# XuehuaOvO/MPC_via_Diffusion_Model

Hardware: AMD Instinct MI355X
Metric: candidate trajectories/sec (100 denoise steps, H=32) (higher is better)
Workload: dtype f32

## Files before the change

### include/mpcd.h

```cpp
#ifndef MPCD_H
#define MPCD_H

#include <stddef.h>
#include <stdint.h>

#ifdef __cplusplus
extern "C" {
#endif

typedef struct mpcd_ctx mpcd_ctx;

enum mpcd_status {
    MPCD_OK = 0,
    MPCD_EINVAL = -1,
    MPCD_EHIP = -2,
    MPCD_ESTATE = -3,
    MPCD_ENOMEM = -4,
    MPCD_EUNSUP = -5,
    MPCD_ENONFINITE = -6,
};

enum mpcd_net_kind {
    MPCD_NET_MLP = 1,
    MPCD_NET_UNET = 2,
// ... 5 lines not shown
    int32_t kind;
    int32_t state_dim;
    int32_t horizon;
    int32_t context_dim;
    int32_t base_dim;
    int32_t n_mults;
    int32_t mults[4];
    int32_t time_emb_dim;
    int32_t cfg_masked;
    int32_t dtype;
} mpcd_net_desc;

int mpcd_net_param_count(const mpcd_net_desc *desc, int32_t *n_tensors, int64_t *n_floats);
int mpcd_net_param_info(const mpcd_net_desc *desc, int32_t i, char *name, size_t name_cap,
                        int32_t *ndim, int64_t shape[4]);

int mpcd_create(int device, mpcd_ctx **out);
void mpcd_destroy(mpcd_ctx *ctx);
const char *mpcd_last_error(void);

int mpcd_load_net(mpcd_ctx *ctx, const mpcd_net_desc *desc, const float *blob_host, size_t n_floats);

int mpcd_set_schedule(mpcd_ctx *ctx, const float *tables_host, int32_t n_steps, const float *posterior_std_host);

enum mpcd_sampler {
    MPCD_DDPM_CFG = 0,
    MPCD_DDIM_CFG = 1,
    MPCD_DDIM = 2,
};

// ... 313 lines not shown
```

### mpc_via_diffusion_model_amd/_native.py

```python
import ctypes
import os

import torch

_HERE = os.path.dirname(os.path.abspath(__file__))
LIB_PATH = os.environ.get("MPCD_LIB") or os.path.join(_HERE, "libmpcd.so")

MPCD_NET_MLP, MPCD_NET_UNET = 1, 2
MPCD_F32, MPCD_F16, MPCD_F32X3, MPCD_F16X2 = 0, 1, 2, 3
MPCD_DDPM_CFG, MPCD_DDIM_CFG, MPCD_DDIM = 0, 1, 2
MPCD_COST_CANONICAL, MPCD_COST_CALMPC = 0, 1
MPCD_COMM_ID_BYTES = 128
MPCD_MAX_ELITES = 64
MPCD_CLIP_CHAIN, MPCD_CLIP_FINAL, MPCD_CLIP_NONE = 0, 1, 2

_STATUS = {-1: "EINVAL", -2: "EHIP", -3: "ESTATE", -4: "ENOMEM", -5: "EUNSUP", -6: "ENONFINITE"}
MPCD_ENONFINITE = -6
MPCD_STEP_CLIPPED, MPCD_STEP_NAN_SAMPLES, MPCD_STEP_NONFINITE_WINNER, MPCD_STEP_F32X3_RERUN = 1, 2, 4, 8
MPCD_STEP_INFEASIBLE = 16
MPCD_MAX_CON_ROWS = 8


class NetDesc(ctypes.Structure):
    _fields_ = [("kind", ctypes.c_int32), ("state_dim", ctypes.c_int32), ("horizon", ctypes.c_int32),
# ... 91 lines not shown
                ("reserved", ctypes.c_int32), ("next_priors_out", ctypes.c_void_p), ("elites_host", ctypes.c_void_p),
                ("elite_viol_host", ctypes.c_void_p), ("viol_host", ctypes.POINTER(ctypes.c_double)),
                ("n_feasible_host", ctypes.POINTER(ctypes.c_int64))]


class TrainCfg(ctypes.Structure):
    _fields_ = [("lr", ctypes.c_float), ("beta1", ctypes.c_float), ("beta2", ctypes.c_float), ("eps", ctypes.c_float),
                ("ema_decay", ctypes.c_float), ("step_start_ema", ctypes.c_int32), ("update_ema_every", ctypes.c_int32)]


EXPORTS = {
    "mpcd_net_param_count": ([ctypes.POINTER(NetDesc), ctypes.POINTER(ctypes.c_int32), ctypes.POINTER(ctypes.c_int64)],
                             ctypes.c_int),
    "mpcd_net_param_info": ([ctypes.POINTER(NetDesc), ctypes.c_int32, ctypes.c_char_p, ctypes.c_size_t,
                             ctypes.POINTER(ctypes.c_int32), ctypes.POINTER(ctypes.c_int64)], ctypes.c_int),
    "mpcd_create": ([ctypes.c_int, ctypes.POINTER(ctypes.c_void_p)], ctypes.c_int),
    "mpcd_destroy": ([ctypes.c_void_p], None),
    "mpcd_last_error": ([], ctypes.c_char_p),
    "mpcd_load_net": ([ctypes.c_void_p, ctypes.POINTER(NetDesc), ctypes.c_void_p, ctypes.c_size_t], ctypes.c_int),
    "mpcd_set_schedule": ([ctypes.c_void_p, ctypes.c_void_p, ctypes.c_int32, ctypes.c_void_p], ctypes.c_int),
    "mpcd_sample_steps": ([ctypes.c_void_p, ctypes.POINTER(SampleArgs), ctypes.POINTER(ctypes.c_int32)], ctypes.c_int),
    "mpcd_sample": ([ctypes.c_void_p, ctypes.POINTER(SampleArgs), ctypes.c_void_p], ctypes.c_int),
    "mpcd_sample_grouped": ([ctypes.c_void_p, ctypes.POINTER(SampleArgs), ctypes.c_int64, ctypes.c_void_p], ctypes.c_int),
    "mpcd_sample_warm": ([ctypes.c_void_p, ctypes.POINTER(SampleArgs), ctypes.c_int64, ctypes.POINTER(WarmStart),
                          ctypes.c_void_p], ctypes.c_int),
    "mpcd_sample_steps_warm": ([ctypes.c_void_p, ctypes.POINTER(SampleArgs), ctypes.POINTER(WarmStart),
                                ctypes.POINTER(ctypes.c_int32)], ctypes.c_int),
    "mpcd_shift_plans": ([ctypes.c_void_p, ctypes.c_void_p, ctypes.c_int64, ctypes.c_int32, ctypes.c_void_p,
                          ctypes.c_int64, ctypes.c_int64, ctypes.c_void_p, ctypes.c_void_p], ctypes.c_int),
    "mpcd_mpc_step_warm": ([ctypes.c_void_p, ctypes.POINTER(StepArgs), ctypes.POINTER(WarmStart), ctypes.c_void_p,
# ... 141 lines not shown
```

### mpc_via_diffusion_model_amd/csrc/internal.h

```cpp
#pragma once
#include <hip/hip_ext.h>
#include <hip/hip_runtime.h>
#include <stdint.h>

#include <mutex>

#include "../../include/mpcd.h"
#include "common.h"

struct CondLayer {
    const float *W;
    const float *b;
    int32_t width;
    int32_t off;
};

void launch_time_prologue(const StepPlan *plan, int n_steps, const float *time_w1, const float *time_b1,
                          const float *time_w2, const float *time_b2, const CondLayer *layers_dev, int n_layers,
                          int cond_dim, int cond_total, float *tproj, hipStream_t stream);

void launch_ctx_prologue(const float *ctx, int64_t n_rows, int ctx_dim, const CondLayer *layers_dev, int n_layers,
                         int cond_dim, int cond_total, float *cproj, hipStream_t stream);
void launch_ctx_replicate(const float *src, int64_t batch, int64_t group, int cond_total, float *dst, hipStream_t stream);
constexpr int kCtxRowMax = 64;
// ... 61 lines not shown
    uint64_t seed;
    int32_t n_steps;
    int32_t mode;
    int32_t clamp_x0;
    float wp1, wf;
    float *dbg;
    int32_t ctx_fused;
    int32_t ctx_dim, n_cond, cond_dim;
    const CondLayer *cond_layers;
    CtxRowArg ctx_row;
    int64_t group;
    int32_t group_wgs;
    int32_t x_init_kind;
    const float *x_init;
    float x_sa, x_sb;
};

int mlp_packed_floats(int d0);
void mlp_pack_weights(int d0, const float *const *lin_w, const float *const *lin_b, float *out);
hipError_t launch_mlp_sampler(int d0, int nb, const MlpSampleArgs &a, hipStream_t stream);
int mlp_packed_floats_x3(int d0);
void mlp_x3_force_layout(int layout);
int mlp_x3_layout_of(int64_t batch, int nb);
int mlp_x3_layout_grouped(int64_t n_groups, int64_t group, int nb);
void mlp_pack_weights_x3(int d0, const float *const *lin_w, const float *const *lin_b, float *out);
hipError_t launch_mlp_x3(int d0, int nb, const MlpSampleArgs &a, hipStream_t stream);
hipError_t launch_mlp_rw(int d0, int rows, int waves, const MlpSampleArgs &a, hipStream_t stream);
bool mlp_h2_supports(int d0, int mode);
int mlp_packed_floats_h2(int d0);
void mlp_pack_weights_h2(int d0, const float *const *lin_w, const float *const *lin_b, float *out);
hipError_t launch_mlp_h2(int d0, int rows, const MlpSampleArgs &a, hipStream_t stream);
// ... 117 lines not shown
```

### mpc_via_diffusion_model_amd/csrc/mlp_common.h

```cpp
#pragma once
#include <hip/hip_runtime.h>
#include <stdint.h>

#include <type_traits>

#include "common.h"

namespace mlpc {

constexpr int NLAYER = 14;
constexpr int COND_TOTAL = 448;
enum { EPI_NONE = 0, EPI_MISH = 1, EPI_CMISH = 2 };
constexpr int MODE_DDPM_XN = 16;

template <int D0>
struct Arch {
    static constexpr int K[NLAYER] = {D0, 32, 32, 64, 64, 128, 128, 128, 256, 64, 128, 32, 32, 32};
    static constexpr int N[NLAYER] = {32, 32, 64, 64, 128, 128, 128, 128, 64, 64, 32, 32, 32, D0};
    __host__ __device__ static constexpr int woff(int l) {
        int o = 0;
        for (int i = 0; i < l; ++i) o += K[i] * N[i] + N[i];
        return o;
    }
    static constexpr int total() { return woff(NLAYER); }
// ... 3 lines not shown
        return o;
    }
    static constexpr int total3() { return woff3(NLAYER); }
    __host__ __device__ static constexpr int boff(int l) {
        int o = 0;
        for (int i = 0; i < l; ++i) o += N[i];
        return o;
    }
    static constexpr int btotal() { return boff(NLAYER); }
};

inline int layer_k(int d0, int l) { return l == 0 ? d0 : Arch<32>::K[l]; }
inline int layer_n(int d0, int l) { return l == NLAYER - 1 ? d0 : Arch<32>::N[l]; }

__host__ __device__ constexpr int cond_off(int j) { return j == 0 ? 0 : j == 1 ? 32 : j == 2 ? 96 : j == 3 ? 224 : j == 4 ? 352 : 416; }

MPCD_DEV StepPlan load_plan(const StepPlan *plan, int s)
{
    typedef const __attribute__((address_space(4))) StepPlan *cplan_t;
    const cplan_t q = (cplan_t)(uintptr_t)plan + s;
    StepPlan r;
    r.t = q->t;
    r.flags = q->flags;
    r.a = q->a;
    r.b = q->b;
    r.c1 = q->c1;
    r.c2 = q->c2;
    r.std = q->std;
    r.sqan = q->sqan;
    r.cn = q->cn;
// ... 152 lines not shown
```

### mpc_via_diffusion_model_amd/csrc/mlp_rw.hip

```cpp
#include <hip/hip_runtime.h>

#include "mlp_x3.h"

namespace {
using namespace mlpx3;
static_assert(WPL == 3, "mlp_rw streams the three-plane pack");

constexpr int RW_W = 4;
constexpr int RW_T = 64 * RW_W;
constexpr int RES_L0 = 5;
constexpr int RES_NL = 3;
constexpr int RES_G = RES_NL * 2 * 4;
constexpr int RES_AG = 21;
constexpr int RES_AG8 = 10;

MPCD_DEV f32x2 exp2_pair(f32x2 z)
{
    float a, b;
    asm("v_exp_f32 %0, %2\n\tv_exp_f32 %1, %3\n\ts_nop 1" : "=&v"(a), "=&v"(b) : "v"(z[0]), "v"(z[1]));
    return f32x2{a, b};
}
MPCD_DEV f32x2 rcp_pair(f32x2 x)
{
    float a, b;
    asm("v_rcp_f32 %0, %2\n\tv_rcp_f32 %1, %3\n\ts_nop 1" : "=&v"(a), "=&v"(b) : "v"(x[0]), "v"(x[1]));
    return f32x2{a, b};
}
MPCD_DEV f32x2 fma2(f32x2 a, f32x2 b, f32x2 c) { return __builtin_elementwise_fma(a, b, c); }

constexpr int wpl(int m) { return m == 0 ? 2 : (m == 1 || m == 3) ? 1 : 0; }
constexpr int xpl(int m) { return (m == 0 || m == 3 || m == 5) ? 0 : (m == 1 || m == 4) ? 1 : 2; }

template <bool FIRST, bool LAST>
MPCD_DEV f32x4 mfma_agpr1(const u32x4 &w, const u32x4 &x, f32x4 acc)
{
    if constexpr (FIRST && LAST)
        asm("s_nop 1\n\tv_mfma_f32_16x16x32_bf16 %0, %1, %2, %0\n\ts_nop 7" : "+v"(acc) : "a"(w), "v"(x));
    else if constexpr (FIRST)
        asm("s_nop 1\n\tv_mfma_f32_16x16x32_bf16 %0, %1, %2, %0" : "+v"(acc) : "a"(w), "v"(x));
    else if constexpr (LAST)
        asm("v_mfma_f32_16x16x32_bf16 %0, %1, %2, %0\n\ts_nop 7" : "+v"(acc) : "a"(w), "v"(x));
    else
        asm("v_mfma_f32_16x16x32_bf16 %0, %1, %2, %0" : "+v"(acc) : "a"(w), "v"(x));
// ... 662 lines not shown
                        !(R == 16 && col >= 8);
        if (ok) nz[0][0] = f32x4{st.z[0], st.z[1], st.z[2], st.z[3]};
    }

    static MPCD_DEV void run(const MlpSampleArgs &p)
    {
        extern __shared__ float lds_f[];
        char *lds = reinterpret_cast<char *>(lds_f);
        const int lane = threadIdx.x & 63;
        const int wave = __builtin_amdgcn_readfirstlane(threadIdx.x >> 6);
        const CandSpan span = cand_span<CPW, GRP>(p.cproj, p.group, p.group_wgs);
        const int64_t cand0 = span.cand0;
        const int n_cand = span.n;
        int lane16 = lane * 16;
        const float *wp = p.wpack;
        float *bi = reinterpret_cast<float *>(lds + L::BI);
        float *bic = reinterpret_cast<float *>(lds + L::BIC);
        float *cps = reinterpret_cast<float *>(lds + L::CPS);

        Res res;
        load_res(res, wp, wave, lane);
        if constexpr (KL8 > 0) {
            constexpr int NT = A::N[8] / 16, KC = A::K[8] / 32, NF = KL8 * NT * 3, NI = (NF + W - 1) / W;
            const __amdgpu_buffer_rsrc_t rs = pack_rsrc(wp);
            u32x4 st[NI];
#pragma unroll
            for (int i = 0; i < NI; ++i) {
                const int f = min(i * W + wave, NF - 1), kc = KS8 + f / (NT * 3), nt = f / 3 % NT, pl = f % 3;
                const int soff = __builtin_amdgcn_readfirstlane(woffx<D0>(8) * 4 + ((nt * KC + kc) * 3 + pl) * 1024);
                st[i] = __builtin_bit_cast(u32x4, __builtin_amdgcn_raw_buffer_load_b128(rs, lane * 16, soff, 0));
            }
#pragma unroll
            for (int i = 0; i < NI; ++i)
                *reinterpret_cast<u32x4 *>(lds + L::W8L + min(i * W + wave, NF - 1) * 1024 + lane * 16) = st[i];
        }
        for (int l = 0; l < NLAYER; ++l)
            for (int i = threadIdx.x; i < A::N[l]; i += NTH) bi[A::boff(l) + i] = wp[woffx<D0>(l) + wfl<D0>(l) + i];
        for (int j = 0; j < 6; ++j)
            for (int i = threadIdx.x; i < A::N[2 * j + 1]; i += NTH)
                bic[cond_off(j) + i] = wp[woffx<D0>(2 * j + 1) + wfl<D0>(2 * j + 1) + i];
        for (int i = threadIdx.x; i < COND_TOTAL; i += NTH)
            cps[i] = !CTX ? 0.f
                          : p.ctx_fused ? ctx_proj_col(p.ctx_row, p.ctx_dim, p.cond_layers, p.n_cond, p.cond_dim, i)
                                        : span.cproj[i];
        if (threadIdx.x < CPW) reinterpret_cast<uint32_t *>(lds + L::AMX)[threadIdx.x] = 0u;
        uint32_t am[2] = {0u, 0u};
        for (int i = threadIdx.x; i < CPW * QUADS; i += NTH) {
            const int c = i / QUADS, qd = i - c * QUADS;
            const int64_t gc = cand0 + c;
            f32x4 z = f32x4{0.f, 0.f, 0.f, 0.f};
            if (in_span<GRP>(p.batch, cand0, n_cand, c)) {
                z = p.noise ? *reinterpret_cast<const f32x4 *>(p.noise + (size_t)gc * D0 + qd * 4)
                            : philox_normal4(p.seed, (uint64_t)(p.global_offset + gc), 0u, (uint32_t)qd);
                if (IS_DDPM && p.x_init) z = warm_x<D0>(p.x_init, p.x_init_kind, p.x_sa, p.x_sb, gc, span.m, qd, z);
                if (p.chain && SMODE != MODE_EPS) *reinterpret_cast<f32x4 *>(p.chain + (size_t)gc * D0 + qd * 4) = z;
            }
            store_x(lds, c, qd * 4, z);
        }
        f32x4 xr[NZT][XG];
        if constexpr (XREG || HEAD_PRE) lds_barrier();
        if constexpr (XREG) load_xr(xr, lds, wave, lane);

        int wofs = 0;
        WS<0> w0;
        load_ws<0>(w0, wp, wave, lane16);
        f32x4 nz[NZT][NB];
        StepPlan sp = load_plan(p.plan, 0);
        if constexpr (W == 4) fetch_noise(nz, p, sp, 0, cand0, n_cand, wave, lane);
        const int tpi = threadIdx.x < COND_TOTAL / 4 ? (int)threadIdx.x : threadIdx.x < COND_TOTAL / 2 ? (int)threadIdx.x - COND_TOTAL / 4 : 0;
        f32x4 tpre = reinterpret_cast<const f32x4 *>(p.tproj)[tpi];
        auto table = [&] {
            if (threadIdx.x < COND_TOTAL / 2) {
                const bool ctx_half = threadIdx.x >= COND_TOTAL / 4;
                const int k = ctx_half ? (int)threadIdx.x - COND_TOTAL / 4 : (int)threadIdx.x;
                f32x4 u = tpre + reinterpret_cast<const f32x4 *>(lds + L::BIC)[k];
                if (ctx_half) u = u + reinterpret_cast<const f32x4 *>(lds + L::CPS)[k];
                reinterpret_cast<f32x4 *>(lds + (ctx_half ? L::TPC : L::TPU))[k] = u;
            }
        };
        if constexpr (HEAD_PRE) {
            table();
            tpre = reinterpret_cast<const f32x4 *>(p.tproj + (size_t)(1 < p.n_steps ? 1 : 0) * COND_TOTAL)[tpi];
        }
        ProfAcc tacc = {};
        const uint64_t rt0 = prof_realtime();
// ... 222 lines not shown
            auto take_noise = [&] {
#pragma unroll
                for (int j = 0; j < NZT; ++j) {
#pragma unroll
                    for (int g = 0; g < NB; ++g) nzc[j][g] = f32x4{0.f, 0.f, 0.f, 0.f};
                    if (IS_DDPM && wave < 4) nzc[j][0] = *reinterpret_cast<const f32x4 *>(lds + L::C0 + ((j * 4 + wave) * 64 + lane) * 16);
                }
            };
            if constexpr (W == 8 && NZT == 1) take_noise();
            bar();
            if constexpr (W == 8 && NZT != 1) take_noise();
            final_and_update(w13, fhd, lds, p, cur, s, cand0, n_cand, nzc, am, xr, wave, lane, tacc);
            if constexpr (W == 8 && W0_LATE) load_ws<0>(w0, ws, wave, lane16);
        }
        MPCD_PROF_DUMP(W, threadIdx.x >> 6, lane);
        if (SMODE != MODE_EPS && SMODE != MODE_EPS1 && p.chain_absmax) {
            const int col = lane & 15;
            store_chain_absmax<CPW, NTH>(reinterpret_cast<uint32_t *>(lds + L::AMX), am, col,
                                          (NB == 2 || R == 16) ? -1 : 16 + col, NB == 1 || R == 32 || col < 8,
                                          p.chain_absmax, cand0, GRP ? cand0 + n_cand : p.batch);
        }
    }
};

template <int D0, int SMODE, bool CTX, int R, int W>
__global__ __launch_bounds__(64 * W, 1) void mlp_rw_kernel(const MlpSampleArgs p)
{
    MlpRw<D0, SMODE, CTX, R, W>::run(p);
}

// ... 41 lines not shown
```

### mpc_via_diffusion_model_amd/csrc/mpcd_api.hip

```cpp
#include <hip/hip_runtime.h>
#include <math.h>
#include <stdarg.h>
#include <stdio.h>
#include <string.h>

#include <algorithm>
#include <atomic>
#include <thread>
#include <cmath>
#include <string>
#include <vector>

#include "../../include/mpcd.h"
#include "comm.h"
#include "train.h"

#include <map>
#include "internal.h"
#include "unet.h"

hipError_t launch_clip_flag(const float *x, int64_t n, int *flag_dev, unsigned *ws, hipStream_t stream);
hipError_t launch_unnormalize(const float *x, int64_t n, int dim, const int *flag_dev, const float *mn_host,
                              const float *mx_host, float *out, hipStream_t stream);
hipError_t launch_rollout_cost(const mpcd_system_desc &d, const double *x0_host, const double *x0_dev, int64_t group,
                               const float *u_norm, const float *umin_host, const float *umax_host, const int *flag_dev,
                               int64_t batch, int H, double *cost, hipStream_t stream,
                               const RolloutSelect *sel = nullptr);
hipError_t launch_clip_flags(const float *x, int64_t n_groups, int64_t group_elems, int *flags_dev, hipStream_t stream);
hipError_t launch_normalize_states(const double *x, int64_t M, int C, const float *mn_host, const float *mx_host,
                                   float *out, hipStream_t stream);
hipError_t launch_control_step(const mpcd_system_desc &d, double *x_dev, int64_t M, int64_t group, const float *u_norm,
                               int H, const double *cost, const float *umin_host, const float *umax_host,
                               const int *flags_dev, int select_first, int decimals, double *u_applied,
// ... 3 lines not shown
                              int64_t n_states, float *out, hipStream_t stream);
hipError_t launch_winner_row(const mpcd_best *best, int64_t lo, int64_t n_local, const float *rows, int row_len,
                             float *out, hipStream_t stream);

int device_cu_count()
{
    constexpr int kMaxDev = 64;
    static std::atomic<int> cu[kMaxDev];
    int dev = 0;
    if (hipGetDevice(&dev) != hipSuccess || dev < 0 || dev >= kMaxDev) return 256;
    int n = cu[dev].load(std::memory_order_relaxed);
    if (n > 0) return n;
    if (hipDeviceGetAttribute(&n, hipDeviceAttributeMultiprocessorCount, dev) != hipSuccess || n <= 0) n = 256;
    cu[dev].store(n, std::memory_order_relaxed);
    return n;
}

namespace {

thread_local std::string g_err;

int fail(int code, const char *fmt, ...) __attribute__((format(printf, 2, 3)));
int fail(int code, const char *fmt, ...)
{
    char buf[512];
    va_list ap;
    va_start(ap, fmt);
    vsnprintf(buf, sizeof buf, fmt, ap);
    va_end(ap);
    g_err = buf;
// ... 177 lines not shown
    }
    template <class T> T *as() const { return static_cast<T *>(p); }
};

}

struct mpcd_ctx {
    int device = 0;
    bool net_loaded = false;
    mpcd_net_desc desc{};
    int cond_dim = 0, cond_total = 0, n_cond = 0;
    DevBuf params;
    DevBuf wpack;
    DevBuf wpack3;
    DevBuf wpackh;
    DevBuf cond_layers;
    UnetWeights unet{};
    bool force_x3 = false;
    DevBuf unet_pack;
    std::vector<float> tables;
    std::vector<float> post_std;
    int n_steps = 0;
    DevBuf plan, tproj, cproj, flag, unet_ws;
    std::vector<StepPlan> plan_host;
    std::vector<StepPlan> plan_cached;
    bool plan_cached_valid = false;
    hipStream_t plan_stream = nullptr;
    hipEvent_t plan_ev = nullptr;
    static constexpr int kEvRing = 256;
    hipEvent_t evr[2][kEvRing] = {};
// ... 104 lines not shown
        out.kind = XINIT_SHARED;
    else if (w->rows == a->batch)
        out.kind = XINIT_PER_CAND;
    else if (group > 0 && a->batch % group == 0 && w->rows == a->batch / group)
        out.kind = XINIT_PER_GROUP;
    else
        return fail(MPCD_EINVAL, "warm start: x_init rows %lld is none of 1, batch %lld%s", (long long)w->rows,
                    (long long)a->batch, group > 0 ? ", batch / group" : "");
    out.x_init = w->x_init;
    out.t_start = w->t_start;
    out.sa = tab(c, T_SQAC, w->t_start - 1);
    out.sb = tab(c, T_SQ1MAC, w->t_start - 1);
    return MPCD_OK;
}

int upload_net(mpcd_ctx *c, const mpcd_net_desc &d, const float *blob, size_t n_floats)
{
    auto spec = param_spec(d);
    size_t total = 0;
    for (auto &p : spec) total += (size_t)p.numel();
    if (n_floats != total) return fail(MPCD_EINVAL, "blob has %zu floats, net needs %zu", n_floats, total);
    std::vector<size_t> off;
    size_t o = 0;
    for (auto &p : spec) {
        off.push_back(o);
        o += (size_t)p.numel();
    }
    auto find = [&](const std::string &n) -> int {
        for (size_t i = 0; i < spec.size(); ++i)
            if (spec[i].name == n) return (int)i;
        return -1;
    };
    int rc = c->params.ensure(total * sizeof(float));
    if (rc) return rc;
    HIP_TRY(hipMemcpy(c->params.p, blob, total * sizeof(float), hipMemcpyHostToDevice));
    const float *dbase = c->params.as<float>();
    auto dptr = [&](const std::string &n) { return dbase + off[find(n)]; };

    std::vector<CondLayer> cl;
    int cond_total = 0;
    for (size_t i = 0; i < spec.size(); ++i) {
        const std::string &n = spec[i].name;
        const std::string suf = ".cond_mlp.1.weight";
        if (n.size() > suf.size() && n.compare(n.size() - suf.size(), suf.size(), suf) == 0) {
            CondLayer L;
            L.W = dbase + off[i];
            L.b = dbase + off[i + 1];
            L.width = (int)spec[i].shape[0];
            L.off = cond_total;
            cond_total += L.width;
            cl.push_back(L);
        }
    }
    if (d.kind == MPCD_NET_MLP) {
        if (cl.size() != 6) return fail(MPCD_EUNSUP, "MLP needs dim_mults of length 3");
        std::vector<CondLayer> ex = {cl[0], cl[1], cl[2], cl[5], cl[3], cl[4]};
        int ofs = 0;
        for (auto &L : ex) {
            L.off = ofs;
            ofs += L.width;
        }
        cl = ex;
        const int d0 = d.horizon * d.state_dim;
        if (d.base_dim != 32 || d.mults[0] != 1 || d.mults[1] != 2 || d.mults[2] != 4 || mlp_packed_floats(d0) < 0)
            return fail(MPCD_EUNSUP, "MLP kernel supports base 32, mults (1,2,4), H*d in {32,64,128}");
        const char *names[14] = {"downs.0.0.blocks.0._network.0", "downs.0.0.blocks.0._network.2",
                                 "downs.1.0.blocks.0._network.0", "downs.1.0.blocks.0._network.2",
                                 "downs.2.0.blocks.0._network.0", "downs.2.0.blocks.0._network.2",
                                 "mid_block1.blocks.0._network.0", "mid_block1.blocks.0._network.2",
                                 "ups.0.0.blocks.0._network.0", "ups.0.0.blocks.0._network.2",
                                 "ups.1.0.blocks.0._network.0", "ups.1.0.blocks.0._network.2",
                                 "final_layer.0._network.0", "final_layer.0._network.2"};
        const float *lw[14], *lb[14];
        for (int l = 0; l < 14; ++l) {
            const int iw = find(std::string(names[l]) + ".weight"), ib = find(std::string(names[l]) + ".bias");
            if (iw < 0 || ib < 0) return fail(MPCD_EINVAL, "missing %s", names[l]);
            lw[l] = blob + off[iw];
            lb[l] = blob + off[ib];
        }
        std::vector<float> packed((size_t)mlp_packed_floats(d0));
        mlp_pack_weights(d0, lw, lb, packed.data());
        rc = c->wpack.ensure(packed.size() * sizeof(float));
        if (rc) return rc;
        HIP_TRY(hipMemcpy(c->wpack.p, packed.data(), packed.size() * sizeof(float), hipMemcpyHostToDevice));
        if (d.dtype == MPCD_F32X3 || d.dtype == MPCD_F16X2) {
            std::vector<float> packed3((size_t)mlp_packed_floats_x3(d0));
            mlp_pack_weights_x3(d0, lw, lb, packed3.data());
            if ((rc = c->wpack3.ensure(packed3.size() * sizeof(float)))) return rc;
            HIP_TRY(hipMemcpy(c->wpack3.p, packed3.data(), packed3.size() * sizeof(float), hipMemcpyHostToDevice));
        }
        if (d.dtype == MPCD_F16X2 && mlp_packed_floats_h2(d0) > 0) {
            std::vector<float> packedh((size_t)mlp_packed_floats_h2(d0));
            mlp_pack_weights_h2(d0, lw, lb, packedh.data());
            if ((rc = c->wpackh.ensure(packedh.size() * sizeof(float)))) return rc;
            HIP_TRY(hipMemcpy(c->wpackh.p, packedh.data(), packedh.size() * sizeof(float), hipMemcpyHostToDevice));
        }
    } else {
        rc = unet_prepare(d, spec.size(), [&](const char *n) -> const float * {
            const int i = find(n);
            return i < 0 ? nullptr : dbase + off[i];
        }, [&](const char *n) -> const float * {
            const int i = find(n);
            return i < 0 ? nullptr : blob + off[i];
        }, c->unet, c->unet_pack.p, c->unet_pack.bytes);
// ... 21 lines not shown
        return MLPK_H2;
    if ((c->desc.dtype == MPCD_F32X3 || c->desc.dtype == MPCD_F16X2) && (shared_ctx || grouped)) return MLPK_X3;
    return MLPK_F32;
}
hipError_t launch_mlp(mpcd_ctx *c, MlpSampleArgs &m, int nb, hipStream_t st)
{
    const int d0 = c->desc.horizon * c->desc.state_dim;
    const int k = mlp_kernel_of(c, m.mode, m.cproj == nullptr || m.cproj_stride == 0, m.group > 0);
    if (k == MLPK_H2) {
        m.wpack = c->wpackh.as<float>();
        const int lay = mlp_x3_layout_of(m.batch, nb);
        return launch_mlp_h2(d0, (lay == 1 || lay == 2 || lay == 4) ? 16 : 32, m, st);
    }
    if (k == MLPK_X3) {
        m.wpack = c->wpack3.as<float>();
        return launch_mlp_x3(d0, nb, m, st);
    }
    m.wpack = c->wpack.as<float>();
    return launch_mlp_sampler(d0, nb, m, st);
}
}

thread_local LaunchEvents g_launch_ev{};

extern "C" {

const char *mpcd_last_error(void) { return g_err.c_str(); }

int mpcd_net_param_count(const mpcd_net_desc *desc, int32_t *n_tensors, int64_t *n_floats)
{
// ... 7 lines not shown
    return MPCD_OK;
}

int mpcd_net_param_info(const mpcd_net_desc *desc, int32_t i, char *name, size_t name_cap, int32_t *ndim,
                        int64_t shape[4])
{
    int rc = check_desc(desc);
    if (rc) return rc;
    auto spec = param_spec(*desc);
    if (i < 0 || i >= (int32_t)spec.size()) return fail(MPCD_EINVAL, "tensor index %d out of range", i);
    const PSpec &p = spec[i];
    if (name && name_cap) snprintf(name, name_cap, "%s", p.name.c_str());
    if (ndim) *ndim = (int32_t)p.shape.size();
    if (shape)
        for (size_t k = 0; k < 4; ++k) shape[k] = k < p.shape.size() ? p.shape[k] : 1;
    return MPCD_OK;
}

int mpcd_create(int device, mpcd_ctx **out)
{
    if (!out) return fail(MPCD_EINVAL, "null out");
    int n = 0;
    HIP_TRY(hipGetDeviceCount(&n));
    if (device < 0 || device >= n) return fail(MPCD_EINVAL, "device %d of %d", device, n);
    DEVICE_GUARD(device);
    auto *c = new mpcd_ctx();
    c->device = device;
    bool ev_ok = hipEventCreateWithFlags(&c->plan_ev, hipEventDisableTiming) == hipSuccess;
    for (int i = 0; i < mpcd_ctx::kEvRing && ev_ok; ++i)
        ev_ok = hipEventCreate(&c->evr[0][i]) == hipSuccess && hipEventCreate(&c->evr[1][i]) == hipSuccess;
// ... 12 lines not shown
        return rc;
    }
    if (hipMemset(c->flag.p, 0, 256) != hipSuccess || hipDeviceSynchronize() != hipSuccess) {
        c->flag.release();
        delete c;
        return fail(MPCD_EHIP, "hipMemset of the reduction counters failed");
    }
    *out = c;
    return MPCD_OK;
}

void mpcd_destroy(mpcd_ctx *c)
{
    if (!c) return;
    DeviceGuard device_guard_(c->device);
    for (DevBuf *b : {&c->params, &c->wpack, &c->wpack3, &c->wpackh, &c->cond_layers, &c->unet_pack, &c->plan, &c->tproj, &c->cproj, &c->flag,
                      &c->unet_ws, &c->step_part, &c->step_out, &c->step_amax, &c->step_elite, &c->loop_ws, &c->loop_cnt,
                      &c->batch_ws, &c->batch_cnt})
        b->release();
    for (int i = 0; i < mpcd_ctx::kEvRing; ++i)
        for (int j = 0; j < 2; ++j)
            if (c->evr[j][i]) (void)hipEventDestroy(c->evr[j][i]);
    if (c->plan_ev) (void)hipEventDestroy(c->plan_ev);
    delete c->comm;
    if (c->step_host) (void)hipHostFree(c->step_host);
    if (c->batch_host) (void)hipHostFree(c->batch_host);
    delete c;
}

int mpcd_load_net(mpcd_ctx *c, const mpcd_net_desc *desc, const float *blob, size_t n_floats)
{
// ... 1730 lines not shown
```

Before: 3.861 million.

## Stage MLP x3 kernel prologue via precomputed launch table with batched loads

Adds a host-built launch table that packs all layer biases, conditioning biases and context-projection weight columns contiguously, and uploads it at net load time. The x3 MLP sampler prologue, for non-(W=4,R=32) configurations, now issues all global loads (table, noise, x_init, residual weights, layer-8 weights) up front as vector loads into registers. It then does the philox and context projection math and writes LDS afterwards, instead of serial scalar loops per layer. This is meant to cut prologue latency from many dependent small global reads. The cost is higher register pressure, extra device memory for the table and a more complex code path.

```diff
diff --git a/include/mpcd.h b/include/mpcd.h
--- a/include/mpcd.h
+++ b/include/mpcd.h
@@ -43,6 +43,8 @@
 int mpcd_net_param_count(const mpcd_net_desc *desc, int32_t *n_tensors, int64_t *n_floats);
 int mpcd_net_param_info(const mpcd_net_desc *desc, int32_t i, char *name, size_t name_cap,
                         int32_t *ndim, int64_t shape[4]);
+int mpcd_mlp_launch_table(const mpcd_net_desc *desc, const float *blob, size_t n_floats, float *pack3,
+                          int64_t *n_pack3, float *table, int64_t *n_table);
 
 int mpcd_create(int device, mpcd_ctx **out);
 void mpcd_destroy(mpcd_ctx *ctx);
diff --git a/mpc_via_diffusion_model_amd/_native.py b/mpc_via_diffusion_model_amd/_native.py
--- a/mpc_via_diffusion_model_amd/_native.py
+++ b/mpc_via_diffusion_model_amd/_native.py
@@ -129,6 +129,9 @@
                              ctypes.c_int),
     "mpcd_net_param_info": ([ctypes.POINTER(NetDesc), ctypes.c_int32, ctypes.c_char_p, ctypes.c_size_t,
                              ctypes.POINTER(ctypes.c_int32), ctypes.POINTER(ctypes.c_int64)], ctypes.c_int),
+    "mpcd_mlp_launch_table": ([ctypes.POINTER(NetDesc), ctypes.c_void_p, ctypes.c_size_t, ctypes.c_void_p,
+                               ctypes.POINTER(ctypes.c_int64), ctypes.c_void_p, ctypes.POINTER(ctypes.c_int64)],
+                              ctypes.c_int),
     "mpcd_create": ([ctypes.c_int, ctypes.POINTER(ctypes.c_void_p)], ctypes.c_int),
     "mpcd_destroy": ([ctypes.c_void_p], None),
     "mpcd_last_error": ([], ctypes.c_char_p),
diff --git a/mpc_via_diffusion_model_amd/csrc/internal.h b/mpc_via_diffusion_model_amd/csrc/internal.h
--- a/mpc_via_diffusion_model_amd/csrc/internal.h
+++ b/mpc_via_diffusion_model_amd/csrc/internal.h
@@ -99,7 +99,10 @@
     int32_t x_init_kind;
     const float *x_init;
     float x_sa, x_sb;
-};
+    const float *ltab;
+};
+
+void mlp_build_launch_table(int d0, int ctx_dim, int cond_dim, const float *pack3, const float *const *cond_w, float *out);
 
 int mlp_packed_floats(int d0);
 void mlp_pack_weights(int d0, const float *const *lin_w, const float *const *lin_b, float *out);
diff --git a/mpc_via_diffusion_model_amd/csrc/mlp_common.h b/mpc_via_diffusion_model_amd/csrc/mlp_common.h
--- a/mpc_via_diffusion_model_amd/csrc/mlp_common.h
+++ b/mpc_via_diffusion_model_amd/csrc/mlp_common.h
@@ -41,6 +41,13 @@
 inline int layer_n(int d0, int l) { return l == NLAYER - 1 ? d0 : Arch<32>::N[l]; }
 
 __host__ __device__ constexpr int cond_off(int j) { return j == 0 ? 0 : j == 1 ? 32 : j == 2 ? 96 : j == 3 ? 224 : j == 4 ? 352 : 416; }
+
+constexpr int ltab_btotal(int d0) { return Arch<32>::boff(NLAYER - 1) + d0; }
+constexpr int LTAB_BI = COND_TOTAL;
+constexpr int ltab_proj(int d0) { return LTAB_BI + ltab_btotal(d0); }
+constexpr int ltab_pstride(int ctx_dim) { return (ctx_dim + 3) & ~3; }
+constexpr int ltab_floats(int d0, int ctx_dim) { return ltab_proj(d0) + COND_TOTAL * ltab_pstride(ctx_dim); }
+static_assert(ltab_btotal(64) == Arch<64>::btotal() && ltab_btotal(128) % 4 == 0 && COND_TOTAL % 4 == 0);
 
 MPCD_DEV StepPlan load_plan(const StepPlan *plan, int s)
 {
diff --git a/mpc_via_diffusion_model_amd/csrc/mlp_rw.hip b/mpc_via_diffusion_model_amd/csrc/mlp_rw.hip
--- a/mpc_via_diffusion_model_amd/csrc/mlp_rw.hip
+++ b/mpc_via_diffusion_model_amd/csrc/mlp_rw.hip
@@ -27,6 +27,10 @@
     return f32x2{a, b};
 }
 MPCD_DEV f32x2 fma2(f32x2 a, f32x2 b, f32x2 c) { return __builtin_elementwise_fma(a, b, c); }
+MPCD_DEV void stg4(float *p, const f32x4 &v)
+{
+    *reinterpret_cast<f32x4 __attribute__((address_space(1))) *>((float __attribute__((address_space(1))) *)p) = v;
+}
 
 constexpr int wpl(int m) { return m == 0 ? 2 : (m == 1 || m == 3) ? 1 : 0; }
 constexpr int xpl(int m) { return (m == 0 || m == 3 || m == 5) ? 0 : (m == 1 || m == 4) ? 1 : 2; }
@@ -719,61 +723,225 @@
         const int n_cand = span.n;
         int lane16 = lane * 16;
         const float *wp = p.wpack;
-        float *bi = reinterpret_cast<float *>(lds + L::BI);
-        float *bic = reinterpret_cast<float *>(lds + L::BIC);
-        float *cps = reinterpret_cast<float *>(lds + L::CPS);
-
+        constexpr bool STAGED = !(W == 4 && R == 32);
         Res res;
-        load_res(res, wp, wave, lane);
-        if constexpr (KL8 > 0) {
-            constexpr int NT = A::N[8] / 16, KC = A::K[8] / 32, NF = KL8 * NT * 3, NI = (NF + W - 1) / W;
-            const __amdgpu_buffer_rsrc_t rs = pack_rsrc(wp);
-            u32x4 st[NI];
-#pragma unroll
-            for (int i = 0; i < NI; ++i) {
-                const int f = min(i * W + wave, NF - 1), kc = KS8 + f / (NT * 3), nt = f / 3 % NT, pl = f % 3;
-                const int soff = __builtin_amdgcn_readfirstlane(woffx<D0>(8) * 4 + ((nt * KC + kc) * 3 + pl) * 1024);
-                st[i] = __builtin_bit_cast(u32x4, __builtin_amdgcn_raw_buffer_load_b128(rs, lane * 16, soff, 0));
-            }
-#pragma unroll
-            for (int i = 0; i < NI; ++i)
-                *reinterpret_cast<u32x4 *>(lds + L::W8L + min(i * W + wave, NF - 1) * 1024 + lane * 16) = st[i];
-        }
-        for (int l = 0; l < NLAYER; ++l)
-            for (int i = threadIdx.x; i < A::N[l]; i += NTH) bi[A::boff(l) + i] = wp[woffx<D0>(l) + wfl<D0>(l) + i];
-        for (int j = 0; j < 6; ++j)
-            for (int i = threadIdx.x; i < A::N[2 * j + 1]; i += NTH)
-                bic[cond_off(j) + i] = wp[woffx<D0>(2 * j + 1) + wfl<D0>(2 * j + 1) + i];
-        for (int i = threadIdx.x; i < COND_TOTAL; i += NTH)
-            cps[i] = !CTX ? 0.f
-                          : p.ctx_fused ? ctx_proj_col(p.ctx_row, p.ctx_dim, p.cond_layers, p.n_cond, p.cond_dim, i)
-                                        : span.cproj[i];
-        if (threadIdx.x < CPW) reinterpret_cast<uint32_t *>(lds + L::AMX)[threadIdx.x] = 0u;
+        WS<0> w0;
+        int wofs = 0;
         uint32_t am[2] = {0u, 0u};
-        for (int i = threadIdx.x; i < CPW * QUADS; i += NTH) {
-            const int c = i / QUADS, qd = i - c * QUADS;
-            const int64_t gc = cand0 + c;
-            f32x4 z = f32x4{0.f, 0.f, 0.f, 0.f};
-            if (in_span<GRP>(p.batch, cand0, n_cand, c)) {
-                z = p.noise ? *reinterpret_cast<const f32x4 *>(p.noise + (size_t)gc * D0 + qd * 4)
-                            : philox_normal4(p.seed, (uint64_t)(p.global_offset + gc), 0u, (uint32_t)qd);
-                if (IS_DDPM && p.x_init) z = warm_x<D0>(p.x_init, p.x_init_kind, p.x_sa, p.x_sb, gc, span.m, qd, z);
-                if (p.chain && SMODE != MODE_EPS) *reinterpret_cast<f32x4 *>(p.chain + (size_t)gc * D0 + qd * 4) = z;
-            }
-            store_x(lds, c, qd * 4, z);
-        }
         f32x4 xr[NZT][XG];
-        if constexpr (XREG || HEAD_PRE) lds_barrier();
-        if constexpr (XREG) load_xr(xr, lds, wave, lane);
-
-        int wofs = 0;
-        WS<0> w0;
-        load_ws<0>(w0, wp, wave, lane16);
         f32x4 nz[NZT][NB];
-        StepPlan sp = load_plan(p.plan, 0);
-        if constexpr (W == 4) fetch_noise(nz, p, sp, 0, cand0, n_cand, wave, lane);
-        const int tpi = threadIdx.x < COND_TOTAL / 4 ? (int)threadIdx.x : threadIdx.x < COND_TOTAL / 2 ? (int)threadIdx.x - COND_TOTAL / 4 : 0;
-        f32x4 tpre = reinterpret_cast<const f32x4 *>(p.tproj)[tpi];
+        StepPlan sp;
+        int tpi;
+        f32x4 tpre;
+#ifdef MPCD_PROF_LAYERS
+        uint64_t t_entry = 0, t_drain = 0;
+#endif
+        if constexpr (STAGED) {
+#ifdef MPCD_PROF_LAYERS
+            t_entry = prof_now();
+#endif
+            const float *a_noise = p.noise, *a_xinit = p.x_init, *a_cps = span.cproj;
+            float *a_chain = p.chain;
+            int a_kind = p.x_init_kind, a_fused = GRP ? 0 : p.ctx_fused, a_cdim = GRP ? 0 : p.ctx_dim;
+            float a_sa = p.x_sa, a_sb = p.x_sb;
+            asm volatile("" : "+s"(a_noise), "+s"(a_xinit), "+s"(a_cps), "+s"(a_chain), "+s"(a_kind), "+s"(a_fused), "+s"(a_cdim),
+                         "+s"(a_sa), "+s"(a_sb));
+            constexpr int PK = 8;
+            float crow[PK];
+            if constexpr (CTX) {
+#pragma unroll
+                for (int k = 0; k < PK; ++k) {
+                    crow[k] = p.ctx_row.v[k];
+                    asm volatile("" : "+s"(crow[k]));
+                }
+            }
+            sp = load_plan(p.plan, 0);
+
+            constexpr int NQB = COND_TOTAL / 4, NQ = NQB + A::btotal() / 4, NTQ = (NQ + NTH - 1) / NTH;
+            static_assert(LTAB_BI == COND_TOTAL && A::btotal() == ltab_btotal(D0) && L::BI % 16 == 0 && L::BIC % 16 == 0);
+            f32x4 tq[NTQ];
+#pragma unroll
+            for (int i = 0; i < NTQ; ++i)
+                tq[i] = ldg4(p.ltab + 4 * min((int)threadIdx.x + i * NTH, NQ - 1));
+            constexpr int NPC = (COND_TOTAL + NTH - 1) / NTH;
+            const float *pj = p.ltab + ltab_proj(D0);
+            const int ps = ltab_pstride(a_cdim);
+            f32x4 pw[NPC][PK / 4];
+            float cpv[NPC], cld[NPC];
+#pragma unroll
+            for (int c = 0; c < NPC; ++c) {
+                cpv[c] = cld[c] = 0.f;
+#pragma unroll
+                for (int u = 0; u < PK / 4; ++u) pw[c][u] = f32x4{0.f, 0.f, 0.f, 0.f};
+            }
+            if constexpr (CTX) {
+#pragma unroll
+                for (int c = 0; c < NPC; ++c) {
+                    const int col = min((int)threadIdx.x + c * NTH, COND_TOTAL - 1);
+                    const float *wc = pj + (size_t)col * ps;
+#pragma unroll
+                    for (int u = 0; u < PK / 4; ++u) pw[c][u] = ldg4(wc + (4 * u < ps ? 4 * u : 0));
+                    cld[c] = *((gptr_f)a_cps + col);
+                }
+            }
+            constexpr int NX = (CPW * QUADS + NTH - 1) / NTH;
+            const bool has_noise = SMODE != MODE_DDPM_CFG && a_noise != nullptr;
+            f32x4 zl[NX], xin[NX];
+            bool xok[NX];
+#pragma unroll
+            for (int j = 0; j < NX; ++j) {
+                const int i = threadIdx.x + j * NTH, c = i / QUADS, qd = i - c * QUADS;
+                const int64_t gc = cand0 + c;
+                xok[j] = i < CPW * QUADS && in_span<GRP>(p.batch, cand0, n_cand, c);
+                if (xok[j] && has_noise) zl[j] = ldg4(a_noise + (size_t)gc * D0 + qd * 4);
+                if (IS_DDPM && xok[j] && a_xinit) {
+                    const int64_t row = a_kind == XINIT_SHARED ? 0 : a_kind == XINIT_PER_CAND ? gc : span.m;
+                    xin[j] = ldg4(a_xinit + (size_t)row * D0 + qd * 4);
+                }
+            }
+            tpi = threadIdx.x < COND_TOTAL / 4 ? (int)threadIdx.x : threadIdx.x < COND_TOTAL / 2 ? (int)threadIdx.x - COND_TOTAL / 4 : 0;
+            tpre = reinterpret_cast<const f32x4 *>(p.tproj)[tpi];
+            auto proj = [&](int c) {
+                double acc = 0.0;
+#pragma unroll
+                for (int k = 0; k < PK; ++k)
+                    if (k < a_cdim) acc += (double)pw[c][k / 4][k % 4] * (double)mish_precise(crow[k]);
+                if (a_cdim > PK) {
+                    const float *wc = pj + (size_t)min((int)threadIdx.x + c * NTH, COND_TOTAL - 1) * ps;
+                    for (int k = PK; k < a_cdim; ++k) acc += (double)*((gptr_f)wc + k) * (double)mish_precise(p.ctx_row.v[k]);
+                }
+                return (float)acc;
+            };
+            if constexpr (CTX) {
+                if (a_fused && a_cdim > PK) {
+#pragma unroll
+                    for (int c = 0; c < NPC; ++c) cpv[c] = proj(c);
+                }
+            }
+            __builtin_amdgcn_sched_barrier(0);
+
+            load_res(res, wp, wave, lane);
+            constexpr int NF8 = KL8 * (A::N[8] / 16) * 3, NI8 = (NF8 + W - 1) / W;
+            u32x4 st[NI8 > 0 ? NI8 : 1];
+            if constexpr (KL8 > 0) {
+                constexpr int NT = A::N[8] / 16, KC = A::K[8] / 32;
+                const __amdgpu_buffer_rsrc_t rs = pack_rsrc(wp);
+#pragma unroll
+                for (int i = 0; i < NI8; ++i) {
+                    const int f = min(i * W + wave, NF8 - 1), kc = KS8 + f / (NT * 3), nt = f / 3 % NT, pl = f % 3;
+                    const int soff = __builtin_amdgcn_readfirstlane(woffx<D0>(8) * 4 + ((nt * KC + kc) * 3 + pl) * 1024);
+                    st[i] = __builtin_bit_cast(u32x4, __builtin_amdgcn_raw_buffer_load_b128(rs, lane * 16, soff, 0));
+                }
+            }
+            load_ws<0>(w0, wp, wave, lane16);
+            __builtin_amdgcn_sched_barrier(0);
+
+            f32x4 zd[NX];
+#pragma unroll
+            for (int j = 0; j < NX; ++j) {
+                const int i = threadIdx.x + j * NTH, c = i / QUADS, qd = i - c * QUADS;
+                zd[j] = f32x4{0.f, 0.f, 0.f, 0.f};
+                if (xok[j] && !has_noise) zd[j] = philox_normal4(p.seed, (uint64_t)(p.global_offset + cand0 + c), 0u, (uint32_t)qd);
+            }
+            if constexpr (CTX) {
+                if (a_fused && a_cdim <= PK) {
+#pragma unroll
+                    for (int c = 0; c < NPC; ++c) cpv[c] = proj(c);
+                }
+                if (!a_fused) {
+#pragma unroll
+                    for (int c = 0; c < NPC; ++c) cpv[c] = cld[c];
+                }
+            }
+            if (threadIdx.x < CPW) reinterpret_cast<uint32_t *>(lds + L::AMX)[threadIdx.x] = 0u;
+            __builtin_amdgcn_sched_barrier(0);
+
+#pragma unroll
+            for (int i = 0; i < NTQ; ++i) {
+                const int qi = threadIdx.x + i * NTH;
+                if (qi < NQ) *reinterpret_cast<f32x4 *>(lds + (qi < NQB ? L::BIC + qi * 16 : L::BI + (qi - NQB) * 16)) = tq[i];
+            }
+#pragma unroll
+            for (int c = 0; c < NPC; ++c) {
+                const int i = threadIdx.x + c * NTH;
+                if (i < COND_TOTAL) reinterpret_cast<float *>(lds + L::CPS)[i] = cpv[c];
+            }
+#pragma unroll
+            for (int j = 0; j < NX; ++j) {
+                const int i = threadIdx.x + j * NTH, c = i / QUADS, qd = i - c * QUADS;
+                if (i >= CPW * QUADS) continue;
+                f32x4 z = zd[j];
+                if (xok[j]) {
+                    if (has_noise) z = zl[j];
+                    if (IS_DDPM && a_xinit) z = q_sample4(a_sa, a_sb, xin[j], z);
+                    if (a_chain && SMODE != MODE_EPS) stg4(a_chain + (size_t)(cand0 + c) * D0 + qd * 4, z);
+                }
+                store_x(lds, c, qd * 4, z);
+            }
+            if constexpr (KL8 > 0) {
+#pragma unroll
+                for (int i = 0; i < NI8; ++i)
+                    *reinterpret_cast<u32x4 *>(lds + L::W8L + min(i * W + wave, NF8 - 1) * 1024 + lane * 16) = st[i];
+            }
+#ifdef MPCD_PROF_LAYERS
+            asm volatile("" ::: "memory");
+            t_drain = prof_now();
+#endif
+            if constexpr (XREG || HEAD_PRE) lds_barrier();
+            if constexpr (XREG) load_xr(xr, lds, wave, lane);
+
+            if constexpr (W == 4) fetch_noise(nz, p, sp, 0, cand0, n_cand, wave, lane);
+        } else {
+            float *bi = reinterpret_cast<float *>(lds + L::BI);
+            float *bic = reinterpret_cast<float *>(lds + L::BIC);
+            float *cps = reinterpret_cast<float *>(lds + L::CPS);
+
+            load_res(res, wp, wave, lane);
+            if constexpr (KL8 > 0) {
+                constexpr int NT = A::N[8] / 16, KC = A::K[8] / 32, NF = KL8 * NT * 3, NI = (NF + W - 1) / W;
+                const __amdgpu_buffer_rsrc_t rs = pack_rsrc(wp);
+                u32x4 st[NI];
+#pragma unroll
+                for (int i = 0; i < NI; ++i) {
+                    const int f = min(i * W + wave, NF - 1), kc = KS8 + f / (NT * 3), nt = f / 3 % NT, pl = f % 3;
+                    const int soff = __builtin_amdgcn_readfirstlane(woffx<D0>(8) * 4 + ((nt * KC + kc) * 3 + pl) * 1024);
+                    st[i] = __builtin_bit_cast(u32x4, __builtin_amdgcn_raw_buffer_load_b128(rs, lane * 16, soff, 0));
+                }
+#pragma unroll
+                for (int i = 0; i < NI; ++i)
+                    *reinterpret_cast<u32x4 *>(lds + L::W8L + min(i * W + wave, NF - 1) * 1024 + lane * 16) = st[i];
+            }
+            for (int l = 0; l < NLAYER; ++l)
+                for (int i = threadIdx.x; i < A::N[l]; i += NTH) bi[A::boff(l) + i] = wp[woffx<D0>(l) + wfl<D0>(l) + i];
+            for (int j = 0; j < 6; ++j)
+                for (int i = threadIdx.x; i < A::N[2 * j + 1]; i += NTH)
+                    bic[cond_off(j) + i] = wp[woffx<D0>(2 * j + 1) + wfl<D0>(2 * j + 1) + i];
+            for (int i = threadIdx.x; i < COND_TOTAL; i += NTH)
+                cps[i] = !CTX ? 0.f
+                              : p.ctx_fused ? ctx_proj_col(p.ctx_row, p.ctx_dim, p.cond_layers, p.n_cond, p.cond_dim, i)
+                                            : span.cproj[i];
+            if (threadIdx.x < CPW) reinterpret_cast<uint32_t *>(lds + L::AMX)[threadIdx.x] = 0u;
+            for (int i = threadIdx.x; i < CPW * QUADS; i += NTH) {
+                const int c = i / QUADS, qd = i - c * QUADS;
+                const int64_t gc = cand0 + c;
+                f32x4 z = f32x4{0.f, 0.f, 0.f, 0.f};
+                if (in_span<GRP>(p.batch, cand0, n_cand, c)) {
+                    z = p.noise ? *reinterpret_cast<const f32x4 *>(p.noise + (size_t)gc * D0 + qd * 4)
+                                : philox_normal4(p.seed, (uint64_t)(p.global_offset + gc), 0u, (uint32_t)qd);
+                    if (IS_DDPM && p.x_init) z = warm_x<D0>(p.x_init, p.x_init_kind, p.x_sa, p.x_sb, gc, span.m, qd, z);
+                    if (p.chain && SMODE != MODE_EPS) *reinterpret_cast<f32x4 *>(p.chain + (size_t)gc * D0 + qd * 4) = z;
+                }
+                store_x(lds, c, qd * 4, z);
+            }
+            if constexpr (XREG || HEAD_PRE) lds_barrier();
+            if constexpr (XREG) load_xr(xr, lds, wave, lane);
+
+            load_ws<0>(w0, wp, wave, lane16);
+            sp = load_plan(p.plan, 0);
+            if constexpr (W == 4) fetch_noise(nz, p, sp, 0, cand0, n_cand, wave, lane);
+            tpi = threadIdx.x < COND_TOTAL / 4 ? (int)threadIdx.x : threadIdx.x < COND_TOTAL / 2 ? (int)threadIdx.x - COND_TOTAL / 4 : 0;
+            tpre = reinterpret_cast<const f32x4 *>(p.tproj)[tpi];
+        }
         auto table = [&] {
             if (threadIdx.x < COND_TOTAL / 2) {
                 const bool ctx_half = threadIdx.x >= COND_TOTAL / 4;
@@ -1026,6 +1194,12 @@
             if constexpr (W == 8 && W0_LATE) load_ws<0>(w0, ws, wave, lane16);
         }
         MPCD_PROF_DUMP(W, threadIdx.x >> 6, lane);
+#ifdef MPCD_PROF_LAYERS
+        if (p.dbg && threadIdx.x == 0 && blockIdx.x < 4096) {
+            p.dbg[32768 + blockIdx.x * 2] = (float)(t_drain - t_entry);
+            p.dbg[32768 + blockIdx.x * 2 + 1] = (float)(ct0 - t_drain);
+        }
+#endif
         if (SMODE != MODE_EPS && SMODE != MODE_EPS1 && p.chain_absmax) {
             const int col = lane & 15;
             store_chain_absmax<CPW, NTH>(reinterpret_cast<uint32_t *>(lds + L::AMX), am, col,
diff --git a/mpc_via_diffusion_model_amd/csrc/mpcd_api.hip b/mpc_via_diffusion_model_amd/csrc/mpcd_api.hip
--- a/mpc_via_diffusion_model_amd/csrc/mpcd_api.hip
+++ b/mpc_via_diffusion_model_amd/csrc/mpcd_api.hip
@@ -17,6 +17,7 @@
 
 #include <map>
 #include "internal.h"
+#include "mlp_common.h"
 #include "unet.h"
 
 hipError_t launch_clip_flag(const float *x, int64_t n, int *flag_dev, unsigned *ws, hipStream_t stream);
@@ -50,6 +51,27 @@
     if (hipDeviceGetAttribute(&n, hipDeviceAttributeMultiprocessorCount, dev) != hipSuccess || n <= 0) n = 256;
     cu[dev].store(n, std::memory_order_relaxed);
     return n;
+}
+
+void mlp_build_launch_table(int d0, int ctx_dim, int cond_dim, const float *pack3, const float *const *cond_w, float *out)
+{
+    using namespace mlpc;
+    std::fill(out, out + ltab_floats(d0, ctx_dim), 0.f);
+    size_t o = 0;
+    int bo = 0;
+    for (int l = 0; l < NLAYER; ++l) {
+        const int K = layer_k(d0, l), N = layer_n(d0, l);
+        o += (size_t)3 * K * N / 2;
+        std::copy(pack3 + o, pack3 + o + N, out + LTAB_BI + bo);
+        if (l % 2 == 1 && l / 2 < 6) std::copy(pack3 + o, pack3 + o + N, out + cond_off(l / 2));
+        o += N;
+        bo += N;
+    }
+    const int ps = ltab_pstride(ctx_dim);
+    for (int j = 0; j < 6; ++j)
+        for (int n = 0; n < layer_n(d0, 2 * j + 1); ++n)
+            for (int k = 0; k < ctx_dim; ++k)
+                out[ltab_proj(d0) + (size_t)(cond_off(j) + n) * ps + k] = cond_w[j][(size_t)n * cond_dim + kCondTdim + k];
 }
 
 namespace {
@@ -257,6 +279,7 @@
     DevBuf wpack;
     DevBuf wpack3;
     DevBuf wpackh;
+    DevBuf ltab;
     DevBuf cond_layers;
     UnetWeights unet{};
     bool force_x3 = false;
@@ -391,6 +414,45 @@
     return MPCD_OK;
 }
 
+bool is_cond_weight(const std::string &n)
+{
+    const std::string suf = ".cond_mlp.1.weight";
+    return n.size() > suf.size() && n.compare(n.size() - suf.size(), suf.size(), suf) == 0;
+}
+
+int mlp_host_tensors(const mpcd_net_desc &d, const std::vector<PSpec> &spec, const std::vector<size_t> &off,
+                     const float *blob, const float **lw, const float **lb, const float **cw)
+{
+    auto find = [&](const std::string &n) -> int {
+        for (size_t i = 0; i < spec.size(); ++i)
+            if (spec[i].name == n) return (int)i;
+        return -1;
+    };
+    const int d0 = d.horizon * d.state_dim;
+    if (d.n_mults != 3 || d.base_dim != 32 || d.mults[0] != 1 || d.mults[1] != 2 || d.mults[2] != 4 || mlp_packed_floats(d0) < 0)
+        return fail(MPCD_EUNSUP, "MLP kernel supports base 32, mults (1,2,4), H*d in {32,64,128}");
+    const char *names[14] = {"downs.0.0.blocks.0._network.0", "downs.0.0.blocks.0._network.2",
+                             "downs.1.0.blocks.0._network.0", "downs.1.0.blocks.0._network.2",
+                             "downs.2.0.blocks.0._network.0", "downs.2.0.blocks.0._network.2",
+                             "mid_block1.blocks.0._network.0", "mid_block1.blocks.0._network.2",
+                             "ups.0.0.blocks.0._network.0", "ups.0.0.blocks.0._network.2",
+                             "ups.1.0.blocks.0._network.0", "ups.1.0.blocks.0._network.2",
+                             "final_layer.0._network.0", "final_layer.0._network.2"};
+    for (int l = 0; l < 14; ++l) {
+        const int iw = find(std::string(names[l]) + ".weight"), ib = find(std::string(names[l]) + ".bias");
+        if (iw < 0 || ib < 0) return fail(MPCD_EINVAL, "missing %s", names[l]);
+        lw[l] = blob + off[iw];
+        lb[l] = blob + off[ib];
+    }
+    std::vector<const float *> cond;
+    for (size_t i = 0; i < spec.size(); ++i)
+        if (is_cond_weight(spec[i].name)) cond.push_back(blob + off[i]);
+    if (cond.size() != 6) return fail(MPCD_EUNSUP, "MLP needs dim_mults of length 3");
+    const int order[6] = {0, 1, 2, 5, 3, 4};
+    for (int j = 0; j < 6; ++j) cw[j] = cond[order[j]];
+    return MPCD_OK;
+}
+
 int upload_net(mpcd_ctx *c, const mpcd_net_desc &d, const float *blob, size_t n_floats)
 {
     auto spec = param_spec(d);
@@ -417,9 +479,7 @@
     std::vector<CondLayer> cl;
     int cond_total = 0;
     for (size_t i = 0; i < spec.size(); ++i) {
-        const std::string &n = spec[i].name;
-        const std::string suf = ".cond_mlp.1.weight";
-        if (n.size() > suf.size() && n.compare(n.size() - suf.size(), suf.size(), suf) == 0) {
+        if (is_cond_weight(spec[i].name)) {
             CondLayer L;
             L.W = dbase + off[i];
             L.b = dbase + off[i + 1];
@@ -439,22 +499,8 @@
         }
         cl = ex;
         const int d0 = d.horizon * d.state_dim;
-        if (d.base_dim != 32 || d.mults[0] != 1 || d.mults[1] != 2 || d.mults[2] != 4 || mlp_packed_floats(d0) < 0)
-            return fail(MPCD_EUNSUP, "MLP kernel supports base 32, mults (1,2,4), H*d in {32,64,128}");
-        const char *names[14] = {"downs.0.0.blocks.0._network.0", "downs.0.0.blocks.0._network.2",
-                                 "downs.1.0.blocks.0._network.0", "downs.1.0.blocks.0._network.2",
-                                 "downs.2.0.blocks.0._network.0", "downs.2.0.blocks.0._network.2",
-                                 "mid_block1.blocks.0._network.0", "mid_block1.blocks.0._network.2",
-                                 "ups.0.0.blocks.0._network.0", "ups.0.0.blocks.0._network.2",
-                                 "ups.1.0.blocks.0._network.0", "ups.1.0.blocks.0._network.2",
-                                 "final_layer.0._network.0", "final_layer.0._network.2"};
-        const float *lw[14], *lb[14];
-        for (int l = 0; l < 14; ++l) {
-            const int iw = find(std::string(names[l]) + ".weight"), ib = find(std::string(names[l]) + ".bias");
-            if (iw < 0 || ib < 0) return fail(MPCD_EINVAL, "missing %s", names[l]);
-            lw[l] = blob + off[iw];
-            lb[l] = blob + off[ib];
-        }
+        const float *lw[14], *lb[14], *cw[6];
+        if ((rc = mlp_host_tensors(d, spec, off, blob, lw, lb, cw))) return rc;
         std::vector<float> packed((size_t)mlp_packed_floats(d0));
         mlp_pack_weights(d0, lw, lb, packed.data());
         rc = c->wpack.ensure(packed.size() * sizeof(float));
@@ -465,6 +511,10 @@
             mlp_pack_weights_x3(d0, lw, lb, packed3.data());
             if ((rc = c->wpack3.ensure(packed3.size() * sizeof(float)))) return rc;
             HIP_TRY(hipMemcpy(c->wpack3.p, packed3.data(), packed3.size() * sizeof(float), hipMemcpyHostToDevice));
+            std::vector<float> tab((size_t)mlpc::ltab_floats(d0, d.context_dim));
+            mlp_build_launch_table(d0, d.context_dim, cond_dim_of(d), packed3.data(), cw, tab.data());
+            if ((rc = c->ltab.ensure(tab.size() * sizeof(float)))) return rc;
+            HIP_TRY(hipMemcpy(c->ltab.p, tab.data(), tab.size() * sizeof(float), hipMemcpyHostToDevice));
         }
         if (d.dtype == MPCD_F16X2 && mlp_packed_floats_h2(d0) > 0) {
             std::vector<float> packedh((size_t)mlp_packed_floats_h2(d0));
@@ -516,6 +566,7 @@
     }
     if (k == MLPK_X3) {
         m.wpack = c->wpack3.as<float>();
+        m.ltab = c->ltab.as<float>();
         return launch_mlp_x3(d0, nb, m, st);
     }
     m.wpack = c->wpack.as<float>();
@@ -553,6 +604,36 @@
     if (ndim) *ndim = (int32_t)p.shape.size();
     if (shape)
         for (size_t k = 0; k < 4; ++k) shape[k] = k < p.shape.size() ? p.shape[k] : 1;
+    return MPCD_OK;
+}
+
+int mpcd_mlp_launch_table(const mpcd_net_desc *desc, const float *blob, size_t n_floats, float *pack3, int64_t *n_pack3,
+                          float *table, int64_t *n_table)
+{
+    int rc = check_desc(desc);
+    if (rc) return rc;
+    if (desc->kind != MPCD_NET_MLP) return fail(MPCD_EINVAL, "mpcd_mlp_launch_table: not an MLP net");
+    auto spec = param_spec(*desc);
+    std::vector<size_t> off;
+    size_t o = 0;
+    for (auto &p : spec) {
+        off.push_back(o);
+        o += (size_t)p.numel();
+    }
+    if (!blob || n_floats != o) return fail(MPCD_EINVAL, "blob has %zu floats, net needs %zu", n_floats, o);
+    const float *lw[14], *lb[14], *cw[6];
+    if ((rc = mlp_host_tensors(*desc, spec, off, blob, lw, lb, cw))) return rc;
+    const int d0 = desc->horizon * desc->state_dim;
+    if (n_pack3) *n_pack3 = mlp_packed_floats_x3(d0);
+    if (n_table) *n_table = mlpc::ltab_floats(d0, desc->context_dim);
+    if (!table) return MPCD_OK;
+    std::vector<float> own;
+    if (!pack3) {
+        own.resize((size_t)mlp_packed_floats_x3(d0));
+        pack3 = own.data();
+    }
+    mlp_pack_weights_x3(d0, lw, lb, pack3);
+    mlp_build_launch_table(d0, desc->context_dim, cond_dim_of(*desc), pack3, cw, table);
     return MPCD_OK;
 }
 
@@ -595,7 +676,7 @@
 {
     if (!c) return;
     DeviceGuard device_guard_(c->device);
-    for (DevBuf *b : {&c->params, &c->wpack, &c->wpack3, &c->wpackh, &c->cond_layers, &c->unet_pack, &c->plan, &c->tproj, &c->cproj, &c->flag,
+    for (DevBuf *b : {&c->params, &c->wpack, &c->wpack3, &c->wpackh, &c->ltab, &c->cond_layers, &c->unet_pack, &c->plan, &c->tproj, &c->cproj, &c->flag,
                       &c->unet_ws, &c->step_part, &c->step_out, &c->step_amax, &c->step_elite, &c->loop_ws, &c->loop_cnt,
                       &c->batch_ws, &c->batch_cnt})
         b->release();
```

Result: faster. 3.923 million, median of 6 (+1.6%).
